# zjwfufu/FateAvatar

Measured on AMD Instinct MI355X. Metric: render+backward frames/sec at 512^2, 100k Gaussians, higher is better.
Workload: dtype f32

## Files before the change

### fateavatar_amd/_lib.py

```python
from __future__ import annotations

import ctypes as C
import os
import subprocess

_HERE = os.path.dirname(os.path.abspath(__file__))
SO_PATH = os.environ.get("FR_HIP_LIB", os.path.join(_HERE, "libfr_hip.so"))

FR_OK = 0
FR_ERR_INVALID_ARGUMENT = 1
FR_ERR_BINNING_CAPACITY = 2
FR_ERR_HIP = 3
FR_ERR_UNSUPPORTED = 4
FR_FLAG_NO_WAIT = 1
FR_FLAG_RAW_ACTIVATIONS = 2
FR_FLAG_FORWARD_ONLY = 4
FR_FLAG_DEPTH_ALPHA = 8
FR_FLAG_CAMERA_GRAD = 16
FR_FLAG_ACCUMULATE_SHIFT = 8
FR_BIND_SHELL = 0
FR_BIND_FACE_LOCAL = 1
FR_BIND_PHONG = 2
FR_BIND_DEFORM = 4

# ... 102 lines not shown
                                   "rotations", "cov3D_precomp", "viewmatrix", "projmatrix", "campos")]


class fr_grads(C.Structure):
    _fields_ = [(n, _fp) for n in ("dL_dmeans2D", "dL_dcolors", "dL_dopacity", "dL_dmeans3D", "dL_dcov3D", "dL_dsh",
                                   "dL_dscales", "dL_drotations")]


class fr_counts(C.Structure):
    _fields_ = [("num_rendered", C.c_uint32), ("num_instances", C.c_uint32), ("max_tile_list", C.c_uint32),
                ("overflow", C.c_uint32)]


EXPORTS = ["fr_create", "fr_destroy", "fr_last_error", "fr_version", "fr_profile_enable", "fr_profile_read", "fr_geometry_bytes", "fr_image_bytes",
           "fr_binning_bytes", "fr_planes_bytes", "fr_camera_grad_workspace_bytes", "fr_forward", "fr_forward_batch", "fr_read_counts", "fr_backward", "fr_backward_batch", "fr_mark_visible", "fr_image_final_T",
           "fr_image_n_contrib", "fr_debug_geometry_field", "fr_debug_binning_region", "fr_debug_selftest_reduce", "fr_knn_workspace_bytes", "fr_knn_mean_dist2", "fr_knn_nearest_dist2", "fr_adam_step", "fr_adam_step_multi", "fr_l1_workspace_bytes", "fr_l1_loss_grad", "fr_l1_loss_grad_batch", "fr_huber_workspace_bytes", "fr_huber_loss_grad", "fr_regularise_workspace_bytes", "fr_gaussian_regularise", "fr_mesh_terms_workspace_bytes", "fr_mesh_terms", "fr_ssim_window", "fr_image_loss_workspace_bytes", "fr_image_loss_grad", "fr_multi_copy", "fr_scaled_sum", "fr_face_scale",
           "fr_bind_forward", "fr_bind_backward", "fr_bind_backward_local", "fr_bind_backward_phong", "fr_bind_backward_deform", "fr_phong_frame", "fr_triwalk", "fr_phong_fit", "fr_texture_corners", "fr_texture_lookup", "fr_texture_lookup_backward",
           "fr_point_lbs_forward", "fr_point_lbs_backward", "fr_point_lbs_pose_workspace_bytes", "fr_point_lbs_backward_pose", "fr_nearest_vertex", "fr_lbs_terms_workspace_bytes", "fr_lbs_terms"]


def build(force: bool = False) -> str:
    cmd = ["make", "-C", os.path.join(_HERE, "csrc"), "-s", "-j8"]
    if force:
        cmd.append("-B")
    subprocess.check_call(cmd)
    return SO_PATH


_lib = None


# ... 40 lines not shown
    L.fr_read_counts.argtypes = [C.c_void_p, C.POINTER(fr_counts)]
    L.fr_read_counts.restype = C.c_int
    L.fr_backward.argtypes = [C.c_void_p, C.POINTER(fr_params), C.POINTER(fr_inputs), _fp, _fp, _fp, _fp, _fp,
                              C.POINTER(fr_grads), C.c_void_p]
    L.fr_backward.restype = C.c_int
    L.fr_mark_visible.argtypes = [C.c_int32, _fp, _fp, _fp, _fp, C.c_void_p]
    L.fr_mark_visible.restype = C.c_int
    L.fr_image_final_T.argtypes = [_fp, C.c_int32, C.c_int32]
    L.fr_image_final_T.restype = C.c_void_p
    L.fr_image_n_contrib.argtypes = [_fp, C.c_int32, C.c_int32]
    L.fr_image_n_contrib.restype = C.c_void_p
    L.fr_debug_geometry_field.argtypes = [_fp, C.c_int32, C.c_int32]
    L.fr_debug_geometry_field.restype = C.c_void_p
    L.fr_debug_binning_region.argtypes = [_fp, C.c_uint64, C.c_int32, C.c_int32, C.c_int32, C.POINTER(C.c_size_t)]
    L.fr_debug_binning_region.restype = C.c_void_p
    L.fr_debug_selftest_reduce.argtypes = [_fp, _fp, C.c_void_p]
    L.fr_debug_selftest_reduce.restype = C.c_int
    L.fr_knn_workspace_bytes.argtypes = [C.c_int32]
    L.fr_knn_workspace_bytes.restype = C.c_size_t
    L.fr_knn_mean_dist2.argtypes = [C.c_int32, _fp, _fp, _fp, C.c_size_t, C.c_void_p]
    L.fr_knn_mean_dist2.restype = C.c_int
    L.fr_knn_nearest_dist2.argtypes = [C.c_int32, _fp, _fp, _fp, C.c_size_t, C.c_void_p]
    L.fr_knn_nearest_dist2.restype = C.c_int
    L.fr_face_scale.argtypes = [C.c_int32, C.c_int32, _fp, _fp, _fp, C.c_void_p]
    L.fr_face_scale.restype = C.c_int
    L.fr_bind_forward.argtypes = [C.POINTER(fr_binding), _fp, _fp, _fp, C.c_void_p]
    L.fr_bind_forward.restype = C.c_int
    L.fr_bind_backward.argtypes = [C.POINTER(fr_binding), _fp, _fp, _fp, _fp, _fp, _fp, _fp, C.c_void_p]
    L.fr_bind_backward.restype = C.c_int
    L.fr_bind_backward_local.argtypes = [C.POINTER(fr_binding), _fp, _fp, _fp, _fp, _fp, _fp, _fp, C.c_void_p]
# ... 139 lines not shown
```

### fateavatar_amd/csrc/fr_api.hip

```cpp
#include "fr_common.hpp"
#include <cstdio>
#include <cstdlib>
#include <cstring>
#include <new>

namespace fr {

thread_local char g_err[512] = "";

int fail_hip(hipError_t e, const char* what, const char* file, int line)
{
    snprintf(g_err, sizeof(g_err), "HIP error %d (%s) at %s:%d in `%s`", (int)e, hipGetErrorString(e), file, line, what);
    return FR_ERR_HIP;
}
int fail_msg(int code, const char* msg)
{
    snprintf(g_err, sizeof(g_err), "%s", msg);
    return code;
}

static int check_binding(const fr_binding* b)
{
    if (!b || b->N < 0 || b->V < 0 || b->F < 0) return fail_msg(FR_ERR_INVALID_ARGUMENT, "fr_binding: null or negative sizes");
    if (b->mode != FR_BIND_SHELL && b->mode != FR_BIND_FACE_LOCAL && b->mode != FR_BIND_PHONG && b->mode != FR_BIND_DEFORM)
// ... 120 lines not shown
    FR_HIP(hipHostGetDevicePointer(reinterpret_cast<void**>(&h->host_counts_dev), h->host_counts, 0));
    FR_HIP(hipEventCreateWithFlags(&h->counts_ready, hipEventDisableTiming));
    FR_HIP(hipEventCreateWithFlags(&h->frame_done, hipEventDisableTiming));
    FR_HIP(hipEventCreateWithFlags(&h->bwd_done, hipEventDisableTiming));
    FR_HIP(hipStreamCreateWithFlags(&h->side_stream, hipStreamNonBlocking));
    FR_HIP(hipEventCreateWithFlags(&h->side_fork, hipEventDisableTiming));
    FR_HIP(hipEventCreateWithFlags(&h->side_join, hipEventDisableTiming));
    const char* bf = getenv("FR_BLEND_FWD");
    h->gather_in_chain = !(bf && strcmp(bf, "gather") == 0);
    const char* pf = getenv("FR_DENSE_PAIRS_FWD");
    const char* pb = getenv("FR_DENSE_PAIRS_BWD");
    h->dense_pairs_fwd = pf ? (uint32_t)strtoul(pf, nullptr, 10) : kDensePairsFwd;
    h->dense_pairs_bwd = pb ? (uint32_t)strtoul(pb, nullptr, 10) : kDensePairsBwd;
    if (const char* hp = getenv("FR_HEAVY_PAIRS")) h->heavy_pairs = (uint32_t)strtoul(hp, nullptr, 10);
    if (const char* cs = getenv("FR_CHAIN_SPINS")) h->chain_spins = (uint32_t)strtoul(cs, nullptr, 10);
    const char* ph = getenv("FR_DEBUG_PAIR_HIST");
    h->debug_pair_hist = ph && ph[0] == '1';
    *out = reinterpret_cast<fr_handle*>(h);
    return FR_OK;
}

int fr_destroy(fr_handle* hh)
{
    fr_handle_impl* h = reinterpret_cast<fr_handle_impl*>(hh);
    if (!h) return FR_OK;
    (void)hipEventDestroy(h->counts_ready);
    if (h->frame_done) (void)hipEventDestroy(h->frame_done);
    if (h->bwd_done) (void)hipEventDestroy(h->bwd_done);
    if (h->side_fork) (void)hipEventDestroy(h->side_fork);
    if (h->side_join) (void)hipEventDestroy(h->side_join);
// ... 83 lines not shown
            return fail_msg(FR_ERR_INVALID_ARGUMENT, "the views of a batch must agree on FR_FLAG_FORWARD_ONLY");
        if ((prm[k]->flags ^ prm[0]->flags) & FR_FLAG_DEPTH_ALPHA)
            return fail_msg(FR_ERR_INVALID_ARGUMENT, "the views of a batch must agree on FR_FLAG_DEPTH_ALPHA");
        if ((prm[k]->flags & FR_FLAG_DEPTH_ALPHA) && (!prm[k]->aux || !prm[k]->aux->out_depth || !prm[k]->aux->out_alpha || !prm[k]->aux->planes))
            return fail_msg(FR_ERR_INVALID_ARGUMENT, "FR_FLAG_DEPTH_ALPHA needs fr_aux::out_depth, out_alpha and planes");
        c[k] = ForwardCall{h, prm[k], in[k], out_color[k], radii[k], geometry[k], image[k], binning[k], binning_capacity[k],
                           counts ? counts + k : nullptr};
    }
    for (int k = 0; k < n_views; k++) {
        c[k].h->last_fwd_flags = prm[k]->flags;
        c[k].h->last_fwd_geometry = geometry[k], c[k].h->last_fwd_binning = binning[k];
    }
    return launch_forward(n_views, c, static_cast<hipStream_t>(stream));
}

int fr_read_counts(fr_handle* hh, fr_counts* counts)
{
    fr_handle_impl* h = reinterpret_cast<fr_handle_impl*>(hh);
    if (!h || !counts) return fail_msg(FR_ERR_INVALID_ARGUMENT, "null argument");
    *counts = *h->host_counts;
    h->counts_seen = true;
    return FR_OK;
}

static int check_backward(const BackwardCall& c, bool batched)
{
    if (!c.h) return fail_msg(FR_ERR_INVALID_ARGUMENT, "null handle");
    int rc = check_frame(c.prm, c.in, false);
    if (rc) return rc;
    if (c.prm->P == 0) return batched ? fail_msg(FR_ERR_INVALID_ARGUMENT, "batched views need P > 0") : FR_OK;
// ... 100 lines not shown
    const ImageView v = ImageView::make(nullptr, W, H);
    const BinningView b = BinningView::make(const_cast<void*>(binning), (size_t)capacity, (size_t)v.tiles_x * v.tiles_y);
    const void* p = nullptr;
    size_t n = 0;
    switch (region) {
        case 0: p = b.masks, n = b.cap * sizeof(uint2); break;
        case 1: p = b.walks, n = b.unit_cap * kUnit * sizeof(uint2); break;
        case 2: p = b.bwd_units, n = b.unit_cap * sizeof(BwdUnit); break;
        case 3: p = b.unit_state, n = b.unit_cap * kUnit * sizeof(float4); break;
        default: return nullptr;
    }
    if (bytes) *bytes = n;
    return p;
}

int fr_debug_selftest_reduce(const float* in, float* out, void* stream)
{
    return launch_selftest_reduce(in, out, static_cast<hipStream_t>(stream));
}

size_t fr_knn_workspace_bytes(int32_t P) { return knn_workspace_bytes(P); }

int fr_knn_mean_dist2(int32_t P, const float* points, float* out, void* workspace, size_t workspace_bytes, void* stream)
{
    if (P < 0 || (P > 0 && (!points || !out || !workspace))) return fail_msg(FR_ERR_INVALID_ARGUMENT, "bad argument");
    return launch_knn(P, points, out, workspace, workspace_bytes, static_cast<hipStream_t>(stream), 0);
}

int fr_knn_nearest_dist2(int32_t P, const float* points, float* out, void* workspace, size_t workspace_bytes, void* stream)
{
// ... 318 lines not shown
```

### fateavatar_amd/csrc/fr_blend_bwd.hip

```cpp
#include "fr_tile.hpp"
#include "fr_diag.hpp"
#include <hip/hip_ext.h>
#include <type_traits>

namespace fr {

#define FR_DPP_ADD(v, ctrl) ((v) + __builtin_bit_cast(float, __builtin_amdgcn_mov_dpp(__builtin_bit_cast(int, (v)), (ctrl), 0xF, 0xF, true)))

__device__ __forceinline__ float swap16_add(float a, float b)
{
    auto r = __builtin_amdgcn_permlane16_swap(__builtin_bit_cast(unsigned, a), __builtin_bit_cast(unsigned, b), false, false);
    return __builtin_bit_cast(float, (unsigned)r[0]) + __builtin_bit_cast(float, (unsigned)r[1]);
}

__device__ __forceinline__ float reduce_scatter_36(const float (&r)[36], int lane)
{
    float a[18], b[9], c[5], d[3], e[2];
    typedef float v2f __attribute__((ext_vector_type(2)));
#pragma unroll
    for (int i = 0; i < 18; i += 2) {
        auto p0 = __builtin_amdgcn_permlane32_swap(__builtin_bit_cast(unsigned, r[2 * i]), __builtin_bit_cast(unsigned, r[2 * i + 1]), false, false);
        auto p1 = __builtin_amdgcn_permlane32_swap(__builtin_bit_cast(unsigned, r[2 * i + 2]), __builtin_bit_cast(unsigned, r[2 * i + 3]), false, false);
        const v2f x = {__builtin_bit_cast(float, (unsigned)p0[0]), __builtin_bit_cast(float, (unsigned)p1[0])};
        const v2f y = {__builtin_bit_cast(float, (unsigned)p0[1]), __builtin_bit_cast(float, (unsigned)p1[1])};
// ... 439 lines not shown
    out[threadIdx.x] = reduce_scatter_36(r, threadIdx.x);
}

int launch_selftest_reduce(const float* in, float* out, hipStream_t s)
{
    hipLaunchKernelGGL(k_selftest_reduce, dim3(1), dim3(64), 0, s, in, out);
    FR_HIP(hipGetLastError());
    return FR_OK;
}

constexpr uint32_t kUnitGrid = 8192;

int launch_blend_backward(int n, const BackwardCall* calls, const GeomView* g, const ImageView* v, bool planes, hipStream_t s, bool debug)
{
    uint32_t unit_grid = 256;
    for (int k = 0; k < n; k++) {
        const fr_handle_impl* h = calls[k].h;
        const uint32_t seen = h->counts_seen ? reinterpret_cast<const uint32_t*>(h->host_counts)[5] : ~0u;
        const uint32_t want = seen > 4u * kUnitGrid ? kUnitGrid : (seen + seen / 8 + kWavesPerWG - 1) / kWavesPerWG;
        unit_grid = min(kUnitGrid, max(unit_grid, want));
    }
    BlendBwdArgs a[kMaxBatch];
    for (int k = 0; k < n; k++) {
        a[k].counts = v[k].counts, a[k].v = v[k], a[k].binning = const_cast<void*>(calls[k].binning);
        a[k].rec_tmpl = g[k].rec_tmpl;
        a[k].W = calls[k].prm->W, a[k].H = calls[k].prm->H, a[k].bg = calls[k].in->background;
        a[k].dL_dpix = calls[k].dL_dpix, a[k].accum = g[k].accum, a[k].dense_pairs = calls[k].h->dense_pairs_bwd;
    }
    if (planes) {
        BlendBwdPlanesArgs ap[kMaxBatch];
        for (int k = 0; k < n; k++) {
            const fr_aux* aux = calls[k].prm->aux;
            ap[k] = BlendBwdPlanesArgs{a[k], BwdPlaneArgs{aux ? aux->dL_ddepth : nullptr, aux ? aux->dL_dalpha : nullptr,
                                                          aux && aux->planes ? PlaneView::make(aux->planes, 0, 0).depth_state : nullptr}};
        }
        StageScope sc(calls[0].h, ST_BLEND_BWD, s);
// ... 17 lines not shown
```

### fateavatar_amd/csrc/fr_blend_fwd.hip

```cpp
#include "fr_tile.hpp"

#ifdef FR_DIAG_FWD_TRACE
namespace fr {
__device__ unsigned long long g_fwd_trace[16384 * 16];
}
extern "C" int fr_debug_read_fwd_trace(void* dst, size_t bytes)
{
    return (int)hipMemcpyFromSymbol(dst, HIP_SYMBOL(fr::g_fwd_trace), bytes < sizeof(fr::g_fwd_trace) ? bytes : sizeof(fr::g_fwd_trace));
}
#define FW_STAMP(K) do { if (lane == 0 && u < 16384u) ::fr::g_fwd_trace[(size_t)u * 16 + (K)] = __builtin_readcyclecounter(); } while (0)
#define FW_STAMPV(K, V) do { if (lane == 0 && u < 16384u) ::fr::g_fwd_trace[(size_t)u * 16 + (K)] = (unsigned long long)(V); } while (0)
#else
#define FW_STAMP(K) do { } while (0)
#define FW_STAMPV(K, V) do { } while (0)
#endif

namespace fr {

__device__ __forceinline__ uint2 footprint_mask(float x0, float y0, float a2, float b2, float c2, float opacity,
                                                float tile_x0, float tile_y0)
{
    const float L = 0.6931471805599453f * __builtin_amdgcn_logf(255.0f * opacity);
    const float far_x = fmaxf(fabsf(x0 - tile_x0), fabsf(x0 - (tile_x0 + 7.f)));
    const float far_y = fmaxf(fabsf(y0 - tile_y0), fabsf(y0 - (tile_y0 + 7.f)));
// ... 464 lines not shown
    uint32_t unit_cap;
    int W, H, tiles_x;
    float* g_tseg;
    float* g_out;
    uint32_t dense_pairs;
    int pair_hist;
    uint32_t* unit_done;
    ImageView v;
    float4* unit_state;
    const float* bg;
    float* out_color;
    uint32_t chain_spins;
};

template <bool FWD_ONLY, bool PLANES>
__device__ __forceinline__ void unit_blend_chained_body(const ChainArgs& a, const PlaneArgs& pl)
{
    DeviceCounts* __restrict__ counts = a.counts;
    const uint4* __restrict__ unit_tile = a.unit_tile;
    const RecSrc recs = a.recs;
    uint2* __restrict__ masks = a.masks;
    const int W = a.W, H = a.H, pair_hist = a.pair_hist;
    float* g_tseg = a.g_tseg;
    float* g_out = a.g_out;
    const uint32_t dense_pairs = a.dense_pairs, chain_spins = a.chain_spins;
    uint32_t* unit_done = a.unit_done;
    const ImageView v = a.v;
    float4* __restrict__ unit_state = a.unit_state;
    const float* __restrict__ bg = a.bg;
    float* __restrict__ out_color = a.out_color;
    __shared__ float4 s_rec_all[kWavesPerWG][kUnit * kRecQuads];
    const int lane = threadIdx.x & 63;
    const int wave_in_wg = __builtin_amdgcn_readfirstlane(threadIdx.x >> 6);
    float4* rec = s_rec_all[wave_in_wg];
    const uint32_t nu_all = counts->num_units;
    const uint32_t u = blockIdx.x * kWavesPerWG + wave_in_wg;
    const uint4 d_early = unit_tile[min(u, a.unit_cap - 1u)];
    asm volatile("" ::"v"(d_early.x), "s"(nu_all));
    if (u >= nu_all) return;
    FW_STAMP(0);
    FW_STAMPV(8, __builtin_amdgcn_s_memrealtime());
    const TransposeConsts tc = transpose_consts(lane);
    const UnitInfo ui = unit_info(d_early, W, H, lane);
    RecRegs rr = fetch_record(recs, (size_t)ui.start, ui.base + (uint32_t)lane, ui.n);
    asm volatile("" ::"v"(rr.q0.x), "v"(rr.q1.x), "v"(rr.q2.x));
    FW_STAMP(1);
    FW_STAMPV(10, ui.n);
    FW_STAMPV(11, ui.seg);
    uint2 fm = make_uint2(0u, 0u);
    if (ui.base + (uint32_t)lane < ui.n) {
        fm = footprint_mask(rr.q0.x, rr.q0.y, rr.q0.z, rr.q0.w, rr.q1.x, rr.q1.y,
                            (float)((int)ui.tx * kTile), (float)((int)ui.ty * kTile));
        if (!PLANES) rr.q2.z = __uint_as_float(fm.x), rr.q2.w = __uint_as_float(fm.y);
        if (!FWD_ONLY) masks[(size_t)ui.start + ui.base + (uint32_t)lane] = fm;
    }
    rec[lane * kRecQuads + 0] = rr.q0;
    rec[lane * kRecQuads + 1] = rr.q1;
    rec[lane * kRecQuads + 2] = rr.q2;
// ... 119 lines not shown
            __hip_atomic_store(o2 + 4 * kUnit, __uint_as_float(rr.lw), __ATOMIC_RELAXED, __HIP_MEMORY_SCOPE_AGENT);
            if (PLANES)
                __hip_atomic_store(pl.unit_depth + (size_t)qq * kUnit + lane, unit_depth_from_memory(unit_tile, recs, qq, tin, fx, fy, ui.inside),
                                   __ATOMIC_RELAXED, __HIP_MEMORY_SCOPE_AGENT);
        }
        asm volatile("s_waitcnt vmcnt(0)" ::: "memory");
    }
    asm volatile("" ::: "memory");
    FW_STAMP(6);
    gather_tile<true, FWD_ONLY, PLANES>(v, ui.ty * (uint32_t)v.tiles_x + ui.tx, u0, ui.seg + 1u, g_out, unit_state, W, H, bg[0], bg[1], bg[2],
                                        out_color, lane, pl);
    FW_STAMP(7);
    FW_STAMPV(12, __builtin_amdgcn_s_memrealtime());
}

__global__ void __launch_bounds__(256) k_unit_blend_chained(ChainArgs a) { unit_blend_chained_body<false, false>(a, PlaneArgs{}); }
__global__ void __launch_bounds__(256) k_unit_blend_chained_batch(BatchOf<ChainArgs> b) { unit_blend_chained_body<false, false>(b.v[blockIdx.y], PlaneArgs{}); }
__global__ void __launch_bounds__(256) k_unit_blend_chained_fwd_only(ChainArgs a) { unit_blend_chained_body<true, false>(a, PlaneArgs{}); }
__global__ void __launch_bounds__(256) k_unit_blend_chained_fwd_only_batch(BatchOf<ChainArgs> b) { unit_blend_chained_body<true, false>(b.v[blockIdx.y], PlaneArgs{}); }
struct ChainPlanesArgs {
    ChainArgs c;
    PlaneArgs p;
};
__global__ void __launch_bounds__(256) k_unit_blend_chained_planes(ChainPlanesArgs a) { unit_blend_chained_body<false, true>(a.c, a.p); }
__global__ void __launch_bounds__(256) k_unit_blend_chained_planes_batch(BatchOf<ChainPlanesArgs> b)
{
    unit_blend_chained_body<false, true>(b.v[blockIdx.y].c, b.v[blockIdx.y].p);
}
__global__ void __launch_bounds__(256) k_unit_blend_chained_fwd_only_planes(ChainPlanesArgs a) { unit_blend_chained_body<true, true>(a.c, a.p); }
__global__ void __launch_bounds__(256) k_unit_blend_chained_fwd_only_planes_batch(BatchOf<ChainPlanesArgs> b)
{
    unit_blend_chained_body<true, true>(b.v[blockIdx.y].c, b.v[blockIdx.y].p);
}

template <bool FWD_ONLY, bool PLANES = false>
__device__ __forceinline__ void tile_gather_body(const DeviceCounts* __restrict__ counts, const ImageView& v,
                                                 const float* __restrict__ g_out, float4* __restrict__ unit_state, int W, int H,
                                                 const float* __restrict__ bg, float* __restrict__ out_color,
                                                 const PlaneArgs& pl = PlaneArgs{})
{
    const uint32_t n_tiles = (uint32_t)v.tiles_x * v.tiles_y;
    const int lane = threadIdx.x & 63;
    const int wave = __builtin_amdgcn_readfirstlane(threadIdx.x >> 6);
    const uint32_t tile = blockIdx.x * kWavesPerWG + wave;
    if (tile >= n_tiles) return;
    const uint32_t overflow = counts->overflow;
    const uint32_t u0 = v.unit_offset[tile];
    const uint32_t n = v.tile_total[tile];
// ... 30 lines not shown

int launch_blend_forward(int n, const FrameView* f, hipStream_t s, bool debug)
{
    fr_handle_impl* h0 = f[0].h;
    const bool fwd_only = (f[0].prm->flags & FR_FLAG_FORWARD_ONLY) != 0;
    const bool planes = (f[0].prm->flags & FR_FLAG_DEPTH_ALPHA) != 0;
    ChainArgs ca[kMaxBatch];
    ChainPlanesArgs cp[kMaxBatch];
    uint32_t unit_wgs = 0, gather_blocks = 0;
    for (int k = 0; k < n; k++) {
        fr_handle_impl* h = f[k].h;
        const fr_params& prm = *f[k].prm;
        const ImageView& v = f[k].v;
        const BinningView& b = f[k].b;
        const uint32_t T = (uint32_t)v.tiles_x * v.tiles_y;
        unit_wgs = max(unit_wgs, (uint32_t)((b.unit_cap + kWavesPerWG - 1) / kWavesPerWG));
        gather_blocks = max(gather_blocks, (T + kWavesPerWG - 1) / kWavesPerWG);
        ChainArgs& c = ca[k];
        c.counts = v.counts, c.unit_tile = b.unit_tile, c.masks = b.masks, c.walks = b.walks, c.bwd_units = b.bwd_units, c.stripe_cursor = b.stripe_cursor, c.heavy_pairs = h->heavy_pairs, c.unit_cap = (uint32_t)b.unit_cap;
        c.recs = RecSrc{b.ids, f[k].g.rec_tmpl};
        c.W = prm.W, c.H = prm.H, c.tiles_x = v.tiles_x, c.g_tseg = b.unit_tseg, c.g_out = b.unit_out;
        c.dense_pairs = h->dense_pairs_fwd, c.pair_hist = h->debug_pair_hist ? 1 : 0;
        c.unit_done = h->gather_in_chain ? b.unit_done : nullptr;
        c.v = v, c.unit_state = b.unit_state, c.bg = f[k].in->background, c.out_color = f[k].out_color;
        c.chain_spins = h->chain_spins;
        if (planes) cp[k] = ChainPlanesArgs{c, PlaneArgs{f[k].pv.unit_depth, f[k].pv.depth_state, f[k].out_depth, f[k].out_alpha}};
    }
    {
        StageScope sc(h0, ST_BLEND_FWD, s);
        if (planes) {
            if (fwd_only) launch_views(k_unit_blend_chained_fwd_only_planes, k_unit_blend_chained_fwd_only_planes_batch, n, cp, unit_wgs, 64 * kWavesPerWG, 0, s);
// ... 17 lines not shown
```

### fateavatar_amd/csrc/fr_common.hpp

```cpp
#pragma once
#include <hip/hip_runtime.h>
#include <stdint.h>
#include <stddef.h>
#include <vector>
#include "../../include/fr_rasterizer.h"

namespace fr {

constexpr int kWave = 64;
constexpr int kTile = 8;
constexpr int kRefTile = 16;
constexpr int kAccumStride = 16;
constexpr int kXcds = 8;
constexpr int kSubWords = 8;
constexpr uint32_t kDensePairsFwd = 1000;
constexpr uint32_t kDensePairsBwd = 1000;
#ifndef FR_PRE_WG
#define FR_PRE_WG 128
#endif
constexpr int kPreWG = FR_PRE_WG;
constexpr uint32_t kBucketCapInit = 64;
constexpr int kSortWaveMax = 256;
constexpr int kSortGroupMax = 2048;
constexpr int kSortRegMax = 4096;
// ... 215 lines not shown
    size_t accum_rows = 0;
    hipEvent_t frame_done = nullptr;
    hipStream_t side_stream = nullptr;
    hipEvent_t side_fork = nullptr, side_join = nullptr;
    hipStream_t last_stream = nullptr;
    bool have_last = false;
    hipEvent_t bwd_done = nullptr;
    hipStream_t last_bwd_stream = nullptr;
    bool have_last_bwd = false;
    bool captured = false;
    std::vector<void*> retired;
    uint32_t dense_pairs_fwd = 0, dense_pairs_bwd = 0;
    bool debug_pair_hist = false;
    uint32_t heavy_pairs = 641;
    uint32_t chain_spins = 1u << 16;
    bool gather_in_chain = true;
    bool profiling = false;
    int32_t last_fwd_flags = 0;
    const void* last_fwd_geometry = nullptr;
    const void* last_fwd_binning = nullptr;
    StageEvents ev[ST_COUNT];
};

struct StageScope {
    fr_handle_impl* h;
    int st;
    hipStream_t s;
    StageScope(fr_handle_impl* h_, int st_, hipStream_t s_) : h(h_), st(st_), s(s_)
    {
        if (!h || !h->profiling) { h = nullptr; return; }
        StageEvents& e = h->ev[st];
        if (e.used == e.start.size()) {
            hipEvent_t a, b;
            if (hipEventCreate(&a) != hipSuccess || hipEventCreate(&b) != hipSuccess) { h = nullptr; return; }
            e.start.push_back(a), e.stop.push_back(b);
        }
        (void)hipEventRecord(e.start[e.used], s);
// ... 291 lines not shown
```

### fateavatar_amd/csrc/fr_tile_sort.hip

```cpp
#include "fr_tile.hpp"

namespace fr {

struct KeySrc {
    const u64* base;
    uint32_t cap;
    uint32_t sub[kXcds];
    __device__ __forceinline__ u64 key(uint32_t i) const
    {
        uint32_t x = 0;
#pragma unroll
        for (int k = 1; k < kXcds; k++) x += (i >= sub[k]) ? 1u : 0u;
        uint32_t s0 = sub[0];
#pragma unroll
        for (int k = 1; k < kXcds; k++) s0 = (x == (uint32_t)k) ? sub[k] : s0;
        return base[(size_t)x * cap + (i - s0)];
    }
};
__device__ __forceinline__ KeySrc key_src(const ImageView& v, uint32_t tile)
{
    KeySrc ks;
    ks.base = reinterpret_cast<const u64*>(v.buckets) + (size_t)tile * kXcds * v.bucket_cap;
    ks.cap = v.bucket_cap;
    const uint4 a = *reinterpret_cast<const uint4*>(v.tile_sub + (size_t)tile * kSubWords);
// ... 156 lines not shown
    for (uint32_t i = tid; i < n; i += nt) {
        const u64 kv = __hip_atomic_load(seg + i, __ATOMIC_RELAXED, __HIP_MEMORY_SCOPE_AGENT);
        ids[start + i] = (uint32_t)kv;
    }
}

__device__ __forceinline__ bool frame_overflow(const DeviceCounts* c, uint32_t bucket_cap)
{
    return c->num_instances > c->capacity || c->max_bucket > bucket_cap;
}

#ifndef FR_MEDIUM_SORTERS
#define FR_MEDIUM_SORTERS 1024
#endif
constexpr uint32_t kMediumSorters = FR_MEDIUM_SORTERS;

struct SortArgs {
    ImageView v;
    uint32_t T, Q;
    u64* keys;
    uint32_t* ids;
    uint4* unit_tile;
    uint32_t unit_cap;
    float* unit_tseg;
    int take_long_lists;
    fr_counts* host_counts;
    uint32_t* unit_done;
    float* empty_color;
    const float* bg;
    int W, H;
    uint32_t* stripe_cursor;
};

template <bool PLANES>
__device__ __forceinline__ void tile_sort_body(const SortArgs& a, float* __restrict__ out_depth, float* __restrict__ out_alpha)
{
    const ImageView v = a.v;
    const uint32_t T = a.T, Q = a.Q, unit_cap = a.unit_cap;
    u64* keys = a.keys;
    uint32_t* ids = a.ids;
    uint4* unit_tile = a.unit_tile;
    float* unit_tseg = a.unit_tseg;
    const int take_long_lists = a.take_long_lists, W = a.W, H = a.H;
    fr_counts* host_counts = a.host_counts;
    uint32_t* unit_done = a.unit_done;
    float* empty_color = a.empty_color;
    const float* __restrict__ bg = a.bg;
    __shared__ SortXchgT<8> sx8;
    SortXchgT<4>& sx = *reinterpret_cast<SortXchgT<4>*>(&sx8);
    const bool overflow = frame_overflow(v.counts, v.bucket_cap);
    if (blockIdx.x == 0 && threadIdx.x < 2 * kStripes) a.stripe_cursor[threadIdx.x * kStripeWords] = 0u;
    if (blockIdx.x == 0 && threadIdx.x == 0) {
        DeviceCounts* c = v.counts;
        c->overflow = overflow ? 1u : 0u;
        host_counts->num_rendered = c->num_rendered;
        host_counts->num_instances = c->num_instances;
        host_counts->max_tile_list = c->max_tile_list;
        host_counts->overflow = overflow ? 1u : 0u;
        reinterpret_cast<uint32_t*>(host_counts)[4] = c->max_bucket;
        reinterpret_cast<uint32_t*>(host_counts)[5] = overflow ? 0u : c->num_units;
        if (overflow) c->num_units = 0u;
    }
    if (blockIdx.x < kMediumSorters) {
        if (overflow) return;
        const int lane = threadIdx.x & 63;
        const int wave = __builtin_amdgcn_readfirstlane(threadIdx.x >> 6);
        const uint32_t nm = v.counts->medium_tiles;
        SortXchgT<2>& sx2 = *reinterpret_cast<SortXchgT<2>*>(&sx);
        for (uint32_t item = blockIdx.x; item < nm; item += kMediumSorters) {
            const uint32_t tile = v.medium_list[item];
            const uint32_t n = v.tile_total[tile];
            int ln = lane, wv = wave;
            asm volatile("" : "+v"(ln), "+s"(wv));
            if (n <= 512u) sort_tile_group<2>(key_src(v, tile), ids, v.tile_offset[tile], n, wv, ln, sx2);
            else if (n <= 1024u) sort_tile_group<4>(key_src(v, tile), ids, v.tile_offset[tile], n, wv, ln, sx);
            else sort_tile_group<8>(key_src(v, tile), ids, v.tile_offset[tile], n, wv, ln, sx8);
        }
        if (take_long_lists) {
            const uint32_t nb = v.counts->big_tiles, nl = v.counts->large_tiles;
            for (uint32_t item = blockIdx.x; item < nb + nl; item += kMediumSorters) {
                const uint32_t tile = item < nb ? v.big_list[item] : v.large_list[item - nb];
                sort_tile_global(key_src(v, tile), keys, ids, v.tile_offset[tile], v.tile_total[tile]);
            }
        }
        return;
    }
    const int lane = threadIdx.x & 63;
    const int wave = __builtin_amdgcn_readfirstlane(threadIdx.x >> 6);
    {
        const uint32_t tile = (uint32_t)wave * Q + (blockIdx.x - kMediumSorters);
        if (blockIdx.x - kMediumSorters < Q && tile < T) {
            const uint32_t start = v.tile_offset[tile];
            const uint32_t n = v.tile_total[tile];
            const uint32_t u0 = v.unit_offset[tile];
            const KeySrc ks = key_src(v, tile);
            asm volatile("" ::"s"(ks.sub[1]), "s"(ks.sub[7]), "s"(start), "s"(n), "s"(u0));
            if (overflow) return;
            const uint32_t nu = (n + kUnit - 1) / kUnit;
            for (uint32_t k = (uint32_t)lane; k < nu; k += 64)
                if (u0 + k < unit_cap)
                    unit_tile[u0 + k] = make_uint4((tile / (uint32_t)v.tiles_x) << 16 | (tile % (uint32_t)v.tiles_x), k, start, n);
            if (unit_tseg)
                for (uint32_t k = 0; k + 1 < nu && u0 + k < unit_cap; k++) unit_tseg[(size_t)(u0 + k) * kUnit + lane] = 0.f;
            if (unit_done)
                for (uint32_t k = (uint32_t)lane; k < nu; k += 64)
                    if (u0 + k < unit_cap) unit_done[u0 + k] = 0u;
// ... 59 lines not shown
        const uint32_t tile = v.large_list[item];
        sort_tile_global(key_src(v, tile), keys, ids, v.tile_offset[tile], v.tile_total[tile]);
    }
}

__global__ void __launch_bounds__(256) k_tile_sort_big(BigSortArgs a) { tile_sort_big_body(a); }
__global__ void __launch_bounds__(256) k_tile_sort_big_batch(BatchOf<BigSortArgs> b) { tile_sort_big_body(b.v[blockIdx.y]); }

int launch_tile_sort(int n, const FrameView* f, hipStream_t s, bool debug)
{
    fr_handle_impl* h0 = f[0].h;
    const bool planes = (f[0].prm->flags & FR_FLAG_DEPTH_ALPHA) != 0;
    SortArgs sa[kMaxBatch];
    BigSortArgs ba[kMaxBatch];
    SortPlanesArgs sp[kMaxBatch];
    uint32_t sort_blocks = 0;
    bool launch_big = false;
    for (int k = 0; k < n; k++) {
        fr_handle_impl* h = f[k].h;
        launch_big = launch_big || !h->counts_seen || h->host_counts->max_tile_list > (uint32_t)kSortGroupMax;
        if (n > 1 && (!h->gather_in_chain || h->gather_in_chain != h0->gather_in_chain))
            return fail_msg(FR_ERR_UNSUPPORTED, "batched frames need the gather inside the forward blend (unset FR_BLEND_FWD)");
    }
    for (int k = 0; k < n; k++) {
        fr_handle_impl* h = f[k].h;
        const fr_params& prm = *f[k].prm;
        const ImageView& v = f[k].v;
        const BinningView& b = f[k].b;
        const uint32_t T = (uint32_t)v.tiles_x * v.tiles_y;
        const uint32_t small_blocks = (T + 3) / 4;
        sort_blocks = max(sort_blocks, small_blocks + kMediumSorters);
        SortArgs& a = sa[k];
        a.v = v, a.T = T, a.Q = small_blocks, a.keys = (u64*)b.keys, a.ids = b.ids, a.unit_tile = b.unit_tile;
        a.unit_cap = (uint32_t)b.unit_cap, a.unit_tseg = b.unit_tseg, a.take_long_lists = launch_big ? 0 : 1;
        a.host_counts = h->host_counts_dev;
        a.unit_done = h->gather_in_chain ? b.unit_done : nullptr;
        a.empty_color = h->gather_in_chain ? f[k].out_color : nullptr;
        a.bg = f[k].in->background, a.W = prm.W, a.H = prm.H, a.stripe_cursor = b.stripe_cursor;
        ba[k].v = v, ba[k].keys = (u64*)b.keys, ba[k].ids = b.ids;
        if (planes) sp[k] = SortPlanesArgs{a, f[k].out_depth, f[k].out_alpha};
    }
    {
        StageScope sc(h0, ST_SORT, s);
        if (launch_big) {
            FR_HIP(hipEventRecord(h0->side_fork, s));
            FR_HIP(hipStreamWaitEvent(h0->side_stream, h0->side_fork, 0));
            launch_views(k_tile_sort_big, k_tile_sort_big_batch, n, ba, kBigSorters, 256, 0, h0->side_stream);
            FR_HIP(hipEventRecord(h0->side_join, h0->side_stream));
        }
        if (planes) launch_views(k_tile_sort_planes, k_tile_sort_planes_batch, n, sp, sort_blocks, 256, 0, s);
        else launch_views(k_tile_sort, k_tile_sort_batch, n, sa, sort_blocks, 256, 0, s);
        for (int k = 0; k < n; k++)
            if (!(f[k].prm->flags & FR_FLAG_NO_WAIT)) FR_HIP(hipEventRecord(f[k].h->counts_ready, s));
        if (launch_big) FR_HIP(hipStreamWaitEvent(s, h0->side_join, 0));
    }
    FR_HIP(hipGetLastError());
// ... 5 lines not shown
```

### include/fr_rasterizer.h

```cpp
#ifndef FR_RASTERIZER_H_INCLUDED
#define FR_RASTERIZER_H_INCLUDED

#include <stddef.h>
#include <stdint.h>

#ifdef __cplusplus
extern "C" {
#endif

#define FR_OK 0
#define FR_ERR_INVALID_ARGUMENT 1
#define FR_ERR_BINNING_CAPACITY 2
#define FR_ERR_HIP 3
#define FR_ERR_UNSUPPORTED 4

typedef struct fr_handle fr_handle;

typedef struct fr_binding fr_binding;

typedef struct fr_aux {
    uint8_t* visible;
    float* grad_accum;
    float* denom;
    const fr_binding* binding;
// ... 234 lines not shown
int fr_texture_lookup(int32_t N, const float* uv, int32_t H, int32_t W, int32_t n_layers, const fr_tex_layer* layers,
                      void* hip_stream);
int fr_texture_lookup_backward(int32_t N, const float* uv, int32_t H, int32_t W, const int32_t* row_start,
                               const int32_t* entries, int32_t n_layers, const fr_tex_layer* layers, void* hip_stream);

int fr_mark_visible(int32_t P, const float* means3D, const float* viewmatrix, const float* projmatrix,
                    uint8_t* present, void* hip_stream);

const float* fr_image_final_T(const void* image, int32_t W, int32_t H);
const uint32_t* fr_image_n_contrib(const void* image, int32_t W, int32_t H);

const void* fr_debug_geometry_field(const void* geometry, int32_t P, int32_t field);

const void* fr_debug_binning_region(const void* binning, uint64_t capacity, int32_t W, int32_t H, int32_t region, size_t* bytes);

int fr_debug_selftest_reduce(const float* in, float* out, void* hip_stream);

size_t fr_knn_workspace_bytes(int32_t P);
int fr_knn_mean_dist2(int32_t P, const float* points, float* out, void* workspace, size_t workspace_bytes,
                      void* hip_stream);
int fr_knn_nearest_dist2(int32_t P, const float* points, float* out, void* workspace, size_t workspace_bytes,
                         void* hip_stream);

#define FR_LBS_MAX_E 64
#define FR_LBS_MAX_J 8
#define FR_LBS_POSE_FEATURES 36
typedef struct fr_pose_state {
    const float* betas;
    const float* pose_feature;
    const float* transforms;
// ... 35 lines not shown
```

Before: 23020.

## Size forward blend and sort grids from previous frame's observed work

The forward chained blend kernel now launches a grid sized from the unit count seen on the previous frame, plus 1/8 slack, rather than the full unit capacity. Each wave loops over units with a grid stride so any extra units are still covered. The tile sort likewise sizes its medium/long-list sorter group from the previous frame's group-list count (minimum 16) instead of a fixed 1024 blocks. This cuts idle workgroup launch and early-exit overhead, at the cost of stale estimates and more serial work per wave when the count grows; debug overrides and inspection entry points are added too.

```diff
diff --git a/fateavatar_amd/_lib.py b/fateavatar_amd/_lib.py
--- a/fateavatar_amd/_lib.py
+++ b/fateavatar_amd/_lib.py
@@ -140,7 +140,7 @@
 
 EXPORTS = ["fr_create", "fr_destroy", "fr_last_error", "fr_version", "fr_profile_enable", "fr_profile_read", "fr_geometry_bytes", "fr_image_bytes",
            "fr_binning_bytes", "fr_planes_bytes", "fr_camera_grad_workspace_bytes", "fr_forward", "fr_forward_batch", "fr_read_counts", "fr_backward", "fr_backward_batch", "fr_mark_visible", "fr_image_final_T",
-           "fr_image_n_contrib", "fr_debug_geometry_field", "fr_debug_binning_region", "fr_debug_selftest_reduce", "fr_knn_workspace_bytes", "fr_knn_mean_dist2", "fr_knn_nearest_dist2", "fr_adam_step", "fr_adam_step_multi", "fr_l1_workspace_bytes", "fr_l1_loss_grad", "fr_l1_loss_grad_batch", "fr_huber_workspace_bytes", "fr_huber_loss_grad", "fr_regularise_workspace_bytes", "fr_gaussian_regularise", "fr_mesh_terms_workspace_bytes", "fr_mesh_terms", "fr_ssim_window", "fr_image_loss_workspace_bytes", "fr_image_loss_grad", "fr_multi_copy", "fr_scaled_sum", "fr_face_scale",
+           "fr_image_n_contrib", "fr_debug_geometry_field", "fr_debug_binning_region", "fr_debug_launch_sizes", "fr_debug_sort_region", "fr_debug_selftest_reduce", "fr_knn_workspace_bytes", "fr_knn_mean_dist2", "fr_knn_nearest_dist2", "fr_adam_step", "fr_adam_step_multi", "fr_l1_workspace_bytes", "fr_l1_loss_grad", "fr_l1_loss_grad_batch", "fr_huber_workspace_bytes", "fr_huber_loss_grad", "fr_regularise_workspace_bytes", "fr_gaussian_regularise", "fr_mesh_terms_workspace_bytes", "fr_mesh_terms", "fr_ssim_window", "fr_image_loss_workspace_bytes", "fr_image_loss_grad", "fr_multi_copy", "fr_scaled_sum", "fr_face_scale",
            "fr_bind_forward", "fr_bind_backward", "fr_bind_backward_local", "fr_bind_backward_phong", "fr_bind_backward_deform", "fr_phong_frame", "fr_triwalk", "fr_phong_fit", "fr_texture_corners", "fr_texture_lookup", "fr_texture_lookup_backward",
            "fr_point_lbs_forward", "fr_point_lbs_backward", "fr_point_lbs_pose_workspace_bytes", "fr_point_lbs_backward_pose", "fr_nearest_vertex", "fr_lbs_terms_workspace_bytes", "fr_lbs_terms"]
 
@@ -211,6 +211,10 @@
     L.fr_debug_geometry_field.restype = C.c_void_p
     L.fr_debug_binning_region.argtypes = [_fp, C.c_uint64, C.c_int32, C.c_int32, C.c_int32, C.POINTER(C.c_size_t)]
     L.fr_debug_binning_region.restype = C.c_void_p
+    L.fr_debug_sort_region.argtypes = [_fp, _fp, C.c_uint64, C.c_int32, C.c_int32, C.c_int32, C.POINTER(C.c_size_t)]
+    L.fr_debug_sort_region.restype = C.c_void_p
+    L.fr_debug_launch_sizes.argtypes = [C.c_void_p, C.c_uint32, C.c_uint32]
+    L.fr_debug_launch_sizes.restype = C.c_int
     L.fr_debug_selftest_reduce.argtypes = [_fp, _fp, C.c_void_p]
     L.fr_debug_selftest_reduce.restype = C.c_int
     L.fr_knn_workspace_bytes.argtypes = [C.c_int32]
diff --git a/fateavatar_amd/csrc/fr_api.hip b/fateavatar_amd/csrc/fr_api.hip
--- a/fateavatar_amd/csrc/fr_api.hip
+++ b/fateavatar_amd/csrc/fr_api.hip
@@ -158,6 +158,8 @@
     h->dense_pairs_bwd = pb ? (uint32_t)strtoul(pb, nullptr, 10) : kDensePairsBwd;
     if (const char* hp = getenv("FR_HEAVY_PAIRS")) h->heavy_pairs = (uint32_t)strtoul(hp, nullptr, 10);
     if (const char* cs = getenv("FR_CHAIN_SPINS")) h->chain_spins = (uint32_t)strtoul(cs, nullptr, 10);
+    if (const char* fw = getenv("FR_FWD_WGS")) h->debug_fwd_wgs = (uint32_t)strtoul(fw, nullptr, 10);
+    if (const char* sg = getenv("FR_SORT_GROUPS")) h->debug_sorters = (uint32_t)strtoul(sg, nullptr, 10);
     const char* ph = getenv("FR_DEBUG_PAIR_HIST");
     h->debug_pair_hist = ph && ph[0] == '1';
     *out = reinterpret_cast<fr_handle*>(h);
@@ -271,6 +273,14 @@
     return launch_forward(n_views, c, static_cast<hipStream_t>(stream));
 }
 
+int fr_debug_launch_sizes(fr_handle* hh, uint32_t forward_workgroups, uint32_t group_sorters)
+{
+    fr_handle_impl* h = reinterpret_cast<fr_handle_impl*>(hh);
+    if (!h) return fail_msg(FR_ERR_INVALID_ARGUMENT, "null handle");
+    h->debug_fwd_wgs = forward_workgroups, h->debug_sorters = group_sorters;
+    return FR_OK;
+}
+
 int fr_read_counts(fr_handle* hh, fr_counts* counts)
 {
     fr_handle_impl* h = reinterpret_cast<fr_handle_impl*>(hh);
@@ -401,6 +411,26 @@
     return p;
 }
 
+const void* fr_debug_sort_region(const void* image, const void* binning, uint64_t capacity, int32_t W, int32_t H, int32_t region, size_t* bytes)
+{
+    if (bytes) *bytes = 0;
+    if (W <= 0 || H <= 0) return nullptr;
+    const ImageView v = ImageView::make(const_cast<void*>(image), W, H);
+    const size_t T = (size_t)v.tiles_x * v.tiles_y;
+    const void* p = nullptr;
+    size_t n = 0;
+    switch (region) {
+        case 0: p = BinningView::make(const_cast<void*>(binning), (size_t)capacity, T).ids, n = (size_t)capacity * sizeof(uint32_t); break;
+        case 1: p = v.tile_offset, n = T * sizeof(uint32_t); break;
+        case 2: p = v.tile_total, n = T * sizeof(uint32_t); break;
+        case 3: p = &v.counts->num_units, n = sizeof(uint32_t); break;
+        case 4: p = &v.counts->capacity, n = sizeof(uint32_t); break;
+        default: return nullptr;
+    }
+    if (bytes) *bytes = n;
+    return p;
+}
+
 int fr_debug_selftest_reduce(const float* in, float* out, void* stream)
 {
     return launch_selftest_reduce(in, out, static_cast<hipStream_t>(stream));
diff --git a/fateavatar_amd/csrc/fr_blend_bwd.hip b/fateavatar_amd/csrc/fr_blend_bwd.hip
--- a/fateavatar_amd/csrc/fr_blend_bwd.hip
+++ b/fateavatar_amd/csrc/fr_blend_bwd.hip
@@ -477,12 +477,7 @@
 int launch_blend_backward(int n, const BackwardCall* calls, const GeomView* g, const ImageView* v, bool planes, hipStream_t s, bool debug)
 {
     uint32_t unit_grid = 256;
-    for (int k = 0; k < n; k++) {
-        const fr_handle_impl* h = calls[k].h;
-        const uint32_t seen = h->counts_seen ? reinterpret_cast<const uint32_t*>(h->host_counts)[5] : ~0u;
-        const uint32_t want = seen > 4u * kUnitGrid ? kUnitGrid : (seen + seen / 8 + kWavesPerWG - 1) / kWavesPerWG;
-        unit_grid = min(kUnitGrid, max(unit_grid, want));
-    }
+    for (int k = 0; k < n; k++) unit_grid = max(unit_grid, wgs_for_seen_work(calls[k].h, kHostWordUnits, kWavesPerWG, kUnitGrid));
     BlendBwdArgs a[kMaxBatch];
     for (int k = 0; k < n; k++) {
         a[k].counts = v[k].counts, a[k].v = v[k], a[k].binning = const_cast<void*>(calls[k].binning);
diff --git a/fateavatar_amd/csrc/fr_blend_fwd.hip b/fateavatar_amd/csrc/fr_blend_fwd.hip
--- a/fateavatar_amd/csrc/fr_blend_fwd.hip
+++ b/fateavatar_amd/csrc/fr_blend_fwd.hip
@@ -502,7 +502,8 @@
 };
 
 template <bool FWD_ONLY, bool PLANES>
-__device__ __forceinline__ void unit_blend_chained_body(const ChainArgs& a, const PlaneArgs& pl)
+__device__ __forceinline__ void unit_blend_chained_unit(const ChainArgs& a, const PlaneArgs& pl, const uint32_t u, const uint32_t nu_all,
+                                                        const uint4 d, float4* rec, const int lane)
 {
     DeviceCounts* __restrict__ counts = a.counts;
     const uint4* __restrict__ unit_tile = a.unit_tile;
@@ -517,19 +518,10 @@
     float4* __restrict__ unit_state = a.unit_state;
     const float* __restrict__ bg = a.bg;
     float* __restrict__ out_color = a.out_color;
-    __shared__ float4 s_rec_all[kWavesPerWG][kUnit * kRecQuads];
-    const int lane = threadIdx.x & 63;
-    const int wave_in_wg = __builtin_amdgcn_readfirstlane(threadIdx.x >> 6);
-    float4* rec = s_rec_all[wave_in_wg];
-    const uint32_t nu_all = counts->num_units;
-    const uint32_t u = blockIdx.x * kWavesPerWG + wave_in_wg;
-    const uint4 d_early = unit_tile[min(u, a.unit_cap - 1u)];
-    asm volatile("" ::"v"(d_early.x), "s"(nu_all));
-    if (u >= nu_all) return;
     FW_STAMP(0);
     FW_STAMPV(8, __builtin_amdgcn_s_memrealtime());
     const TransposeConsts tc = transpose_consts(lane);
-    const UnitInfo ui = unit_info(d_early, W, H, lane);
+    const UnitInfo ui = unit_info(d, W, H, lane);
     RecRegs rr = fetch_record(recs, (size_t)ui.start, ui.base + (uint32_t)lane, ui.n);
     asm volatile("" ::"v"(rr.q0.x), "v"(rr.q1.x), "v"(rr.q2.x));
     FW_STAMP(1);
@@ -679,24 +671,50 @@
     FW_STAMPV(12, __builtin_amdgcn_s_memrealtime());
 }
 
-__global__ void __launch_bounds__(256) k_unit_blend_chained(ChainArgs a) { unit_blend_chained_body<false, false>(a, PlaneArgs{}); }
-__global__ void __launch_bounds__(256) k_unit_blend_chained_batch(BatchOf<ChainArgs> b) { unit_blend_chained_body<false, false>(b.v[blockIdx.y], PlaneArgs{}); }
-__global__ void __launch_bounds__(256) k_unit_blend_chained_fwd_only(ChainArgs a) { unit_blend_chained_body<true, false>(a, PlaneArgs{}); }
-__global__ void __launch_bounds__(256) k_unit_blend_chained_fwd_only_batch(BatchOf<ChainArgs> b) { unit_blend_chained_body<true, false>(b.v[blockIdx.y], PlaneArgs{}); }
 struct ChainPlanesArgs {
     ChainArgs c;
     PlaneArgs p;
 };
-__global__ void __launch_bounds__(256) k_unit_blend_chained_planes(ChainPlanesArgs a) { unit_blend_chained_body<false, true>(a.c, a.p); }
-__global__ void __launch_bounds__(256) k_unit_blend_chained_planes_batch(BatchOf<ChainPlanesArgs> b)
-{
-    unit_blend_chained_body<false, true>(b.v[blockIdx.y].c, b.v[blockIdx.y].p);
-}
-__global__ void __launch_bounds__(256) k_unit_blend_chained_fwd_only_planes(ChainPlanesArgs a) { unit_blend_chained_body<true, true>(a.c, a.p); }
-__global__ void __launch_bounds__(256) k_unit_blend_chained_fwd_only_planes_batch(BatchOf<ChainPlanesArgs> b)
-{
-    unit_blend_chained_body<true, true>(b.v[blockIdx.y].c, b.v[blockIdx.y].p);
-}
+__device__ __forceinline__ const ChainArgs& chain_of(const ChainArgs& a) { return a; }
+__device__ __forceinline__ const ChainArgs& chain_of(const ChainPlanesArgs& a) { return a.c; }
+__device__ __forceinline__ PlaneArgs planes_of(const ChainArgs&) { return PlaneArgs{}; }
+__device__ __forceinline__ PlaneArgs planes_of(const ChainPlanesArgs& a) { return a.p; }
+
+template <bool FWD_ONLY, bool PLANES, typename A>
+__device__ __forceinline__ void unit_blend_chained_body(const A* views, const uint32_t view)
+{
+    const ChainArgs& a0 = chain_of(views[view]);
+    const uint4* __restrict__ unit_tile = a0.unit_tile;
+    const uint32_t unit_cap = a0.unit_cap;
+    __shared__ float4 s_rec_all[kWavesPerWG][kUnit * kRecQuads];
+    const uint32_t nu_all = a0.counts->num_units;
+    uint32_t u = blockIdx.x * kWavesPerWG + __builtin_amdgcn_readfirstlane(threadIdx.x >> 6);
+    uint4 d = unit_tile[min(u, unit_cap - 1u)];
+    asm volatile("" ::"v"(d.x), "s"(nu_all));
+    if (u >= nu_all) return;
+    const uint32_t covered = gridDim.x * kWavesPerWG;
+    const uint32_t nu_end = min(nu_all, unit_cap);
+    for (;;) {
+        int ln = threadIdx.x & 63, wv = __builtin_amdgcn_readfirstlane(threadIdx.x >> 6);
+        uint32_t vw = view;
+        asm volatile("" : "+v"(ln), "+s"(wv), "+s"(vw));
+        unit_blend_chained_unit<FWD_ONLY, PLANES>(chain_of(views[vw]), planes_of(views[vw]), u, nu_all, d, s_rec_all[wv], ln);
+        if (u >= nu_end || nu_end - u <= covered) break;
+        u += covered;
+        d = unit_tile[u];
+        __builtin_amdgcn_fence(__ATOMIC_ACQ_REL, "wavefront");
+        __builtin_amdgcn_wave_barrier();
+    }
+}
+
+__global__ void __launch_bounds__(256) k_unit_blend_chained(ChainArgs a) { unit_blend_chained_body<false, false>(&a, 0u); }
+__global__ void __launch_bounds__(256) k_unit_blend_chained_batch(BatchOf<ChainArgs> b) { unit_blend_chained_body<false, false>(b.v, blockIdx.y); }
+__global__ void __launch_bounds__(256) k_unit_blend_chained_fwd_only(ChainArgs a) { unit_blend_chained_body<true, false>(&a, 0u); }
+__global__ void __launch_bounds__(256) k_unit_blend_chained_fwd_only_batch(BatchOf<ChainArgs> b) { unit_blend_chained_body<true, false>(b.v, blockIdx.y); }
+__global__ void __launch_bounds__(256) k_unit_blend_chained_planes(ChainPlanesArgs a) { unit_blend_chained_body<false, true>(&a, 0u); }
+__global__ void __launch_bounds__(256) k_unit_blend_chained_planes_batch(BatchOf<ChainPlanesArgs> b) { unit_blend_chained_body<false, true>(b.v, blockIdx.y); }
+__global__ void __launch_bounds__(256) k_unit_blend_chained_fwd_only_planes(ChainPlanesArgs a) { unit_blend_chained_body<true, true>(&a, 0u); }
+__global__ void __launch_bounds__(256) k_unit_blend_chained_fwd_only_planes_batch(BatchOf<ChainPlanesArgs> b) { unit_blend_chained_body<true, true>(b.v, blockIdx.y); }
 
 template <bool FWD_ONLY, bool PLANES = false>
 __device__ __forceinline__ void tile_gather_body(const DeviceCounts* __restrict__ counts, const ImageView& v,
@@ -757,7 +775,9 @@
         const ImageView& v = f[k].v;
         const BinningView& b = f[k].b;
         const uint32_t T = (uint32_t)v.tiles_x * v.tiles_y;
-        unit_wgs = max(unit_wgs, (uint32_t)((b.unit_cap + kWavesPerWG - 1) / kWavesPerWG));
+        const uint32_t cap_wgs = (uint32_t)((b.unit_cap + kWavesPerWG - 1) / kWavesPerWG);
+        const uint32_t want = h->debug_fwd_wgs ? min(h->debug_fwd_wgs, cap_wgs) : wgs_for_seen_work(h, kHostWordUnits, kWavesPerWG, cap_wgs);
+        unit_wgs = max(unit_wgs, max(want, 1u));
         gather_blocks = max(gather_blocks, (T + kWavesPerWG - 1) / kWavesPerWG);
         ChainArgs& c = ca[k];
         c.counts = v.counts, c.unit_tile = b.unit_tile, c.masks = b.masks, c.walks = b.walks, c.bwd_units = b.bwd_units, c.stripe_cursor = b.stripe_cursor, c.heavy_pairs = h->heavy_pairs, c.unit_cap = (uint32_t)b.unit_cap;
diff --git a/fateavatar_amd/csrc/fr_common.hpp b/fateavatar_amd/csrc/fr_common.hpp
--- a/fateavatar_amd/csrc/fr_common.hpp
+++ b/fateavatar_amd/csrc/fr_common.hpp
@@ -253,6 +253,7 @@
     bool debug_pair_hist = false;
     uint32_t heavy_pairs = 641;
     uint32_t chain_spins = 1u << 16;
+    uint32_t debug_fwd_wgs = 0, debug_sorters = 0;
     bool gather_in_chain = true;
     bool profiling = false;
     int32_t last_fwd_flags = 0;
@@ -260,6 +261,18 @@
     const void* last_fwd_binning = nullptr;
     StageEvents ev[ST_COUNT];
 };
+
+constexpr int kHostWordMaxBucket = 4;
+constexpr int kHostWordUnits = 5;
+constexpr int kHostWordGroupLists = 6;
+
+static inline uint32_t wgs_for_seen_work(const fr_handle_impl* h, int word, uint32_t per_wg, uint32_t cap_wgs)
+{
+    if (!h->counts_seen || h->host_counts->overflow) return cap_wgs;
+    const uint64_t seen = reinterpret_cast<const uint32_t*>(h->host_counts)[word];
+    const uint64_t want = (seen + seen / 8 + per_wg - 1) / per_wg;
+    return want < cap_wgs ? (uint32_t)want : cap_wgs;
+}
 
 struct StageScope {
     fr_handle_impl* h;
diff --git a/fateavatar_amd/csrc/fr_tile_sort.hip b/fateavatar_amd/csrc/fr_tile_sort.hip
--- a/fateavatar_amd/csrc/fr_tile_sort.hip
+++ b/fateavatar_amd/csrc/fr_tile_sort.hip
@@ -194,10 +194,12 @@
 #define FR_MEDIUM_SORTERS 1024
 #endif
 constexpr uint32_t kMediumSorters = FR_MEDIUM_SORTERS;
+constexpr uint32_t kMinSorters = 16;
 
 struct SortArgs {
     ImageView v;
     uint32_t T, Q;
+    uint32_t sorters;
     u64* keys;
     uint32_t* ids;
     uint4* unit_tile;
@@ -216,7 +218,7 @@
 __device__ __forceinline__ void tile_sort_body(const SortArgs& a, float* __restrict__ out_depth, float* __restrict__ out_alpha)
 {
     const ImageView v = a.v;
-    const uint32_t T = a.T, Q = a.Q, unit_cap = a.unit_cap;
+    const uint32_t T = a.T, Q = a.Q, unit_cap = a.unit_cap, sorters = a.sorters;
     u64* keys = a.keys;
     uint32_t* ids = a.ids;
     uint4* unit_tile = a.unit_tile;
@@ -237,17 +239,18 @@
         host_counts->num_instances = c->num_instances;
         host_counts->max_tile_list = c->max_tile_list;
         host_counts->overflow = overflow ? 1u : 0u;
-        reinterpret_cast<uint32_t*>(host_counts)[4] = c->max_bucket;
-        reinterpret_cast<uint32_t*>(host_counts)[5] = overflow ? 0u : c->num_units;
+        reinterpret_cast<uint32_t*>(host_counts)[kHostWordMaxBucket] = c->max_bucket;
+        reinterpret_cast<uint32_t*>(host_counts)[kHostWordUnits] = overflow ? 0u : c->num_units;
+        reinterpret_cast<uint32_t*>(host_counts)[kHostWordGroupLists] = c->medium_tiles + (take_long_lists ? c->big_tiles + c->large_tiles : 0u);
         if (overflow) c->num_units = 0u;
     }
-    if (blockIdx.x < kMediumSorters) {
+    if (blockIdx.x < sorters) {
         if (overflow) return;
         const int lane = threadIdx.x & 63;
         const int wave = __builtin_amdgcn_readfirstlane(threadIdx.x >> 6);
         const uint32_t nm = v.counts->medium_tiles;
         SortXchgT<2>& sx2 = *reinterpret_cast<SortXchgT<2>*>(&sx);
-        for (uint32_t item = blockIdx.x; item < nm; item += kMediumSorters) {
+        for (uint32_t item = blockIdx.x; item < nm; item += sorters) {
             const uint32_t tile = v.medium_list[item];
             const uint32_t n = v.tile_total[tile];
             int ln = lane, wv = wave;
@@ -258,7 +261,7 @@
         }
         if (take_long_lists) {
             const uint32_t nb = v.counts->big_tiles, nl = v.counts->large_tiles;
-            for (uint32_t item = blockIdx.x; item < nb + nl; item += kMediumSorters) {
+            for (uint32_t item = blockIdx.x; item < nb + nl; item += sorters) {
                 const uint32_t tile = item < nb ? v.big_list[item] : v.large_list[item - nb];
                 sort_tile_global(key_src(v, tile), keys, ids, v.tile_offset[tile], v.tile_total[tile]);
             }
@@ -268,8 +271,8 @@
     const int lane = threadIdx.x & 63;
     const int wave = __builtin_amdgcn_readfirstlane(threadIdx.x >> 6);
     {
-        const uint32_t tile = (uint32_t)wave * Q + (blockIdx.x - kMediumSorters);
-        if (blockIdx.x - kMediumSorters < Q && tile < T) {
+        const uint32_t tile = (uint32_t)wave * Q + (blockIdx.x - sorters);
+        if (blockIdx.x - sorters < Q && tile < T) {
             const uint32_t start = v.tile_offset[tile];
             const uint32_t n = v.tile_total[tile];
             const uint32_t u0 = v.unit_offset[tile];
@@ -359,7 +362,7 @@
     SortArgs sa[kMaxBatch];
     BigSortArgs ba[kMaxBatch];
     SortPlanesArgs sp[kMaxBatch];
-    uint32_t sort_blocks = 0;
+    uint32_t small_blocks_max = 0, sorters = 0;
     bool launch_big = false;
     for (int k = 0; k < n; k++) {
         fr_handle_impl* h = f[k].h;
@@ -374,7 +377,10 @@
         const BinningView& b = f[k].b;
         const uint32_t T = (uint32_t)v.tiles_x * v.tiles_y;
         const uint32_t small_blocks = (T + 3) / 4;
-        sort_blocks = max(sort_blocks, small_blocks + kMediumSorters);
+        small_blocks_max = max(small_blocks_max, small_blocks);
+        const uint32_t want = h->debug_sorters ? min(h->debug_sorters, kMediumSorters)
+                                               : max(kMinSorters, wgs_for_seen_work(h, kHostWordGroupLists, 1u, kMediumSorters));
+        sorters = max(sorters, want);
         SortArgs& a = sa[k];
         a.v = v, a.T = T, a.Q = small_blocks, a.keys = (u64*)b.keys, a.ids = b.ids, a.unit_tile = b.unit_tile;
         a.unit_cap = (uint32_t)b.unit_cap, a.unit_tseg = b.unit_tseg, a.take_long_lists = launch_big ? 0 : 1;
@@ -383,8 +389,12 @@
         a.empty_color = h->gather_in_chain ? f[k].out_color : nullptr;
         a.bg = f[k].in->background, a.W = prm.W, a.H = prm.H, a.stripe_cursor = b.stripe_cursor;
         ba[k].v = v, ba[k].keys = (u64*)b.keys, ba[k].ids = b.ids;
-        if (planes) sp[k] = SortPlanesArgs{a, f[k].out_depth, f[k].out_alpha};
-    }
+    }
+    for (int k = 0; k < n; k++) {
+        sa[k].sorters = sorters;
+        if (planes) sp[k] = SortPlanesArgs{sa[k], f[k].out_depth, f[k].out_alpha};
+    }
+    const uint32_t sort_blocks = small_blocks_max + sorters;
     {
         StageScope sc(h0, ST_SORT, s);
         if (launch_big) {
diff --git a/include/fr_rasterizer.h b/include/fr_rasterizer.h
--- a/include/fr_rasterizer.h
+++ b/include/fr_rasterizer.h
@@ -272,6 +272,11 @@
 
 const void* fr_debug_binning_region(const void* binning, uint64_t capacity, int32_t W, int32_t H, int32_t region, size_t* bytes);
 
+const void* fr_debug_sort_region(const void* image, const void* binning, uint64_t capacity, int32_t W, int32_t H, int32_t region,
+                                 size_t* bytes);
+
+int fr_debug_launch_sizes(fr_handle* h, uint32_t forward_workgroups, uint32_t group_sorters);
+
 int fr_debug_selftest_reduce(const float* in, float* out, void* hip_stream);
 
 size_t fr_knn_workspace_bytes(int32_t P);
```

Result: faster. 23520 (median of 5 runs) (+2.2%).
